# waczjoan/gaussian-mesh-splatting

Measured on AMD Instinct MI355X. Metric: train iters/s (fwd+bwd raster) @800×800, 300k Gaussians; HBM GB/s vs roofline, higher is better.
Workload: dtype f32

## Files before the change

gaussian-mesh-splatting_amd/csrc/blend_micro.hip:

```cpp
#include <stdlib.h>

#include "gms_common.h"
#include "gms_blend.h"
#include "gms_segments.h"

namespace gms {

struct MPix {
    int xi, yi, tid, b; bool inside; float xf, yf;
    static __device__ __forceinline__ MPix of_tile(const BlendGrid &g, int tile);
};

__device__ __forceinline__ MPix micro_pixel(const BlendGrid &g, int tx, int ty, int b, int li)
{
    MPix p;
    p.b = b;
    p.xi = tx * TILE + (b & 3) * 4 + (li & 3);
    p.yi = ty * TILE + (b >> 2) * 4 + (li >> 2);
    p.inside = p.xi < g.W && p.yi < g.H;
    p.xf = (float)p.xi; p.yf = (float)p.yi;
    p.tid = b * 16 + li;
    return p;
}

__device__ __forceinline__ uint32_t max4rows(uint32_t v)
{
    const uint32_t a = (uint32_t)__builtin_amdgcn_readlane((int)v, 0), b = (uint32_t)__builtin_amdgcn_readlane((int)v, 16);
    const uint32_t c = (uint32_t)__builtin_amdgcn_readlane((int)v, 32), d = (uint32_t)__builtin_amdgcn_readlane((int)v, 48);
    return max(max(a, b), max(c, d));
}

constexpr int LMAX = 256;

__device__ __forceinline__ MPix MPix::of_tile(const BlendGrid &g, int tile)
{
    return micro_pixel(g, tile % g.gx, tile / g.gx, (int)(threadIdx.x >> 4), (int)(threadIdx.x & 15));
}

__global__ void __launch_bounds__(BLOCK) micro_tloc_check_kernel(BlendGrid g)
{
    tile_dead_check<MPix>(g);
}

__global__ void __launch_bounds__(BLOCK) micro_finalize_kernel(BlendGrid g, BlendFwdOut o)
{
    const uint32_t order_blocks = g.bwd_order ? UNIT_ORDER_CLASSES : 0u;
    if (blockIdx.x < order_blocks) {
        __shared__ UnitOrderLds S;
        const uint32_t n = min(g.unit_first[g.T], g.max_units);
        unit_order_partition(blockIdx.x, n, blend_grid_units(g.max_units), g.order_on ? UNIT_ORDER_CLASSES : 0u,
                             [&](uint32_t i) { return (uint32_t)g.unit_cost[i]; },
                             [&](uint32_t i) { const uint2 r = reinterpret_cast<const uint2 *>(g.unit_tile)[4 * (size_t)i + 2]; return r.x != r.y; },
                             g.bwd_order, S);
        return;
    }
    finalize_tile<8, MPix>(g, o, (int)(blockIdx.x - order_blocks));
}

struct Phases {
    unsigned long long *buf; bool on;
    __device__ __forceinline__ Phases(const BlendGrid &g, uint32_t bit = 1024u) : buf(nullptr), on(false)
    {
        if (dbg_on(g, bit) && g.dbg_buf) {
            buf = g.dbg_buf + 8ull * 65536ull * (threadIdx.x >> 6) + 8ull * (blockIdx.x & 65535u);
            on = (threadIdx.x & 63) == 0;
        }
    }
    __device__ __forceinline__ void mark(int k) { if (on) buf[k] = wall_clock64(); }
    __device__ __forceinline__ void value(int k, unsigned long long v) { if (on) buf[k] = v; }
};

template <int CTRL>
__device__ __forceinline__ float dpp_mov(float v)
{
    return __builtin_bit_cast(float, __builtin_amdgcn_update_dpp(0, __builtin_bit_cast(int, v), CTRL, 0xf, 0xf, false));
}

#define GMS_BANK_PAIR(D, A, B, CTRL, LO, HI)                                                                                          \
    "v_add_f32_dpp " D ", " A ", " A " " CTRL " row_mask:0xf bank_mask:" LO "\n\tv_add_f32_dpp " D ", " B ", " B " " CTRL " row_mask:0xf bank_mask:" HI "\n\t"
template <bool NINE>
__device__ __forceinline__ void bank_stage_ror8(const float *v, float (&u)[5])
{
    if (NINE)
        asm volatile("s_nop 1\n\t"
                     GMS_BANK_PAIR("%0", "%5", "%10", "row_ror:8", "0x3", "0xc") GMS_BANK_PAIR("%1", "%6", "%11", "row_ror:8", "0x3", "0xc")
                     GMS_BANK_PAIR("%2", "%7", "%12", "row_ror:8", "0x3", "0xc") GMS_BANK_PAIR("%3", "%8", "%13", "row_ror:8", "0x3", "0xc")
                     "v_add_f32_dpp %4, %9, %9 row_ror:8 row_mask:0xf bank_mask:0x3\n\t"
                     : "=&v"(u[0]), "=&v"(u[1]), "=&v"(u[2]), "=&v"(u[3]), "=&v"(u[4])
                     : "v"(v[0]), "v"(v[1]), "v"(v[2]), "v"(v[3]), "v"(v[4]), "v"(v[5]), "v"(v[6]), "v"(v[7]), "v"(v[8]));
    else
        asm volatile("s_nop 1\n\t"
                     GMS_BANK_PAIR("%0", "%5", "%10", "row_ror:8", "0x3", "0xc") GMS_BANK_PAIR("%1", "%6", "%11", "row_ror:8", "0x3", "0xc")
                     GMS_BANK_PAIR("%2", "%7", "%12", "row_ror:8", "0x3", "0xc") GMS_BANK_PAIR("%3", "%8", "%13", "row_ror:8", "0x3", "0xc")
                     GMS_BANK_PAIR("%4", "%9", "%14", "row_ror:8", "0x3", "0xc")
                     : "=&v"(u[0]), "=&v"(u[1]), "=&v"(u[2]), "=&v"(u[3]), "=&v"(u[4])
                     : "v"(v[0]), "v"(v[1]), "v"(v[2]), "v"(v[3]), "v"(v[4]), "v"(v[5]), "v"(v[6]), "v"(v[7]), "v"(v[8]), "v"(v[9]));
}
__device__ __forceinline__ void bank_stage_half_mirror(float a0, float b0, float a1, float b1, float &w0, float &w1)
{
    asm volatile("s_nop 1\n\t"
                 GMS_BANK_PAIR("%0", "%2", "%3", "row_half_mirror", "0x5", "0xa") GMS_BANK_PAIR("%1", "%4", "%5", "row_half_mirror", "0x5", "0xa")
                 : "=&v"(w0), "=&v"(w1) : "v"(a0), "v"(b0), "v"(a1), "v"(b1));
}

template <bool NINE = false>
__device__ __forceinline__ float row_reduce10(const float *v, bool b1, bool b0)
{
    float u[5];
    bank_stage_ror8<NINE>(v, u);
    float w0, w1;
    bank_stage_half_mirror(u[0], u[3], u[1], u[4], w0, w1);
    const float w2 = u[2] + dpp_mov<0x141>(u[2]);
    const float x0 = (b1 ? w1 : w0) + dpp_mov<0x4E>(b1 ? w0 : w1);
    const float x1 = w2 + dpp_mov<0x4E>(w2);
    return (b0 ? x1 : x0) + dpp_mov<0xB1>(b0 ? x0 : x1);
}

template <int CTRL, int ROW_MASK = 0xf>
__device__ __forceinline__ float dpp_max(float v)
{
    return fmaxf(v, __builtin_bit_cast(float, __builtin_amdgcn_update_dpp(0, __builtin_bit_cast(int, v), CTRL, ROW_MASK, 0xf, false)));
}
__device__ __forceinline__ float wave_max_to_lane63(float v)
{
    v = dpp_max<0xB1>(v); v = dpp_max<0x4E>(v); v = dpp_max<0x141>(v); v = dpp_max<0x140>(v);
    v = dpp_max<0x142, 0xa>(v); v = dpp_max<0x143, 0xc>(v);
    return v;
}

template <bool WITHD> struct RecTail { using type = float2; };
template <> struct RecTail<false> { using type = float; };
__device__ __forceinline__ void set_tail(float2 &d, float b, float invd) { d = make_float2(b, invd); }
__device__ __forceinline__ void set_tail(float &d, float b, float) { d = b; }
__device__ __forceinline__ float2 get_tail(const float2 &d) { return d; }
__device__ __forceinline__ float2 get_tail(const float &d) { return make_float2(d, 0.f); }
struct __attribute__((aligned(16))) WideTail { float2 v; float2 unused; };
__device__ __forceinline__ void set_tail(WideTail &d, float b, float invd) { d.v = make_float2(b, invd); }
__device__ __forceinline__ float2 get_tail(const WideTail &d) { return d.v; }
template <bool WITHD, bool WIDE> struct RecTailSel { using type = typename RecTail<WITHD>::type; };
template <> struct RecTailSel<true, true> { using type = WideTail; };
template <bool WITHD, bool WIDE = false>
struct UnitRecsT {
    float4 ra[LMAX];
    float4 rb[LMAX];
    typename RecTailSel<WITHD, WIDE>::type rc[LMAX];
    uint8_t list[16][LMAX];
    uint16_t ocnt[16];
    uint8_t order[16];
    uint8_t wcnt4[16][4];
};
using UnitRecs = UnitRecsT<true, true>;

template <int NE> __device__ __forceinline__ uint32_t list_load(const uint8_t *lst, uint32_t pos);
template <> __device__ __forceinline__ uint32_t list_load<2>(const uint8_t *lst, uint32_t pos) { return *reinterpret_cast<const uint16_t *>(lst + pos); }
template <> __device__ __forceinline__ uint32_t list_load<4>(const uint8_t *lst, uint32_t pos) { return *reinterpret_cast<const uint32_t *>(lst + pos); }

template <bool FILTER, bool WITHD, bool WIDE>
__device__ __forceinline__ uint32_t unit_stage(const BlendGrid &g, const Unit &u, UnitRecsT<WITHD, WIDE> &S, const SplatRec *rec, uint32_t *cmax_out,
                                               Phases *ph = nullptr)
{
    const int tid = threadIdx.x, lane = tid & 63, wave = tid >> 6;
    const uint32_t cn = u.end - u.beg;
    uint16_t *mm = g.mmask;
    uint32_t mask = 0, id = 0;
    float cm = 0.f;
    if ((uint32_t)tid < cn) {
        id = reinterpret_cast<const uint32_t *>(g.keys)[2 * (size_t)(u.beg + tid)];
        if (!FILTER) mask = mm[u.beg + tid];
        const SplatRec r = rec[id];
        if (FILTER) { mask = block_mask(r, (float)(u.tx * TILE), (float)(u.ty * TILE)); mm[u.beg + tid] = (uint16_t)mask; }
        S.ra[tid] = r.q0; S.rb[tid] = r.q1; set_tail(S.rc[tid], r.q2.x, r.q2.y);
        cm = fmaxf(fmaxf(fabsf(r.q1.z), fabsf(r.q1.w)), fabsf(r.q2.x));
    } else if (tid < LMAX) {
        S.ra[tid] = make_float4(0.f, 0.f, 0.f, 0.f); S.rb[tid] = make_float4(0.f, 0.f, 0.f, 0.f); set_tail(S.rc[tid], 0.f, 0.f);
    }
    if (cmax_out) {
        cm = wave_max_to_lane63(cm);
        if (lane == 63 && cm > 0.f) atomicMax(cmax_out, __float_as_uint(cm));
    }
    if (GMS_EXPERIMENTS && ph) { __builtin_amdgcn_s_waitcnt(0); ph->mark(3); }
    uint64_t bal[16];
    uint32_t mycnt = 0;
#pragma unroll
    for (int b = 0; b < 16; b++) {
        bal[b] = __ballot((mask >> b) & 1u);
        const uint32_t n = (uint32_t)__builtin_popcountll(bal[b]);
        asm("v_writelane_b32 %0, %1, %2" : "+v"(mycnt) : "s"(n), "n"(b));
    }
    if (lane < 16) S.wcnt4[lane][wave] = (uint8_t)mycnt;
    __syncthreads();
    if (GMS_EXPERIMENTS && ph) ph->mark(4);
    const uint32_t w4 = *reinterpret_cast<const uint32_t *>(&S.wcnt4[lane & 15][0]);
    const uint32_t basev = __builtin_amdgcn_sad_u8(w4 & ((1u << (8 * wave)) - 1u), 0u, 0u);
#pragma unroll
    for (int b = 0; b < 16; b++) {
        const uint32_t base = (uint32_t)__builtin_amdgcn_readlane((int)basev, b);
        const uint32_t pos = __builtin_amdgcn_mbcnt_hi((uint32_t)(bal[b] >> 32), __builtin_amdgcn_mbcnt_lo((uint32_t)bal[b], base));
        if ((mask >> b) & 1u) S.list[b][pos] = (uint8_t)tid;
    }
    if (tid < 16) {
        const uint32_t c = __builtin_amdgcn_sad_u8(w4, 0u, 0u);
        uint32_t rank = 0;
#pragma unroll
        for (int s0 = 0; s0 < 16; s0++) {
            const uint32_t cs = (uint32_t)__builtin_amdgcn_readlane((int)c, s0);
            rank += (cs > c || (cs == c && s0 < tid)) ? 1u : 0u;
        }
        S.order[rank] = (uint8_t)tid; S.ocnt[rank] = (uint16_t)c;
        if (FILTER && rank == 0) g.unit_cost[u.idx] = (uint16_t)c;
    }
    __syncthreads();
    return id;
}

constexpr uint32_t LAST_NONE = 0x7fffffffu;
constexpr int REM_STOPPED = -0x40000000;
template <int E>
__device__ __forceinline__ void fwd_step_exec(float pw, float al, float cr, float cg, float cb, float cd, float &T, float &C0, float &C1, float &C2,
                                              float &Dp, int &rem, uint32_t &last)
{
    uint64_t sv; float tmp, w;
    asm volatile("s_mov_b64 %[sv], exec\n\t"
                 "v_cmpx_lt_i32_e32 vcc, %[e], %[rem]\n\t"
                 "v_cmpx_ge_f32_e32 vcc, 0, %[pw]\n\t"
                 "v_cmpx_le_f32_e32 vcc, %[amin], %[al]\n\t"
                 "v_sub_f32_e32 %[tmp], 1.0, %[al]\n\t"
                 "v_mul_f32_e32 %[tmp], %[T], %[tmp]\n\t"
                 "v_cmp_ngt_f32_e32 vcc, %[tmin], %[tmp]\n\t"
                 "v_cndmask_b32_e32 %[rem], %[stopped], %[rem], vcc\n\t"
                 "s_and_b64 exec, exec, vcc\n\t"
                 "v_mul_f32_e32 %[w], %[al], %[T]\n\t"
                 "v_fmac_f32_e32 %[C0], %[cr], %[w]\n\t"
                 "v_fmac_f32_e32 %[C1], %[cg], %[w]\n\t"
                 "v_fmac_f32_e32 %[C2], %[cb], %[w]\n\t"
                 "v_fmac_f32_e32 %[Dp], %[cd], %[w]\n\t"
                 "v_mov_b32_e32 %[T], %[tmp]\n\t"
                 "v_sub_u32_e32 %[last], %[e], %[rem]\n\t"
                 "s_mov_b64 exec, %[sv]"
                 : [sv] "=&s"(sv), [tmp] "=&v"(tmp), [w] "=&v"(w), [T] "+v"(T), [C0] "+v"(C0), [C1] "+v"(C1), [C2] "+v"(C2), [Dp] "+v"(Dp),
                   [rem] "+v"(rem), [last] "+v"(last)
                 : [e] "n"(E), [pw] "v"(pw), [al] "v"(al), [amin] "s"(ALPHA_MIN), [tmin] "s"(T_MIN), [stopped] "v"(REM_STOPPED), [cr] "v"(cr), [cg] "v"(cg), [cb] "v"(cb), [cd] "v"(cd)
                 : "vcc");
}
template <int E>
__device__ __forceinline__ void tloc_step_exec(float pw, float al, float &Tl, int rem)
{
    uint64_t sv; float tmp;
    asm volatile("s_mov_b64 %[sv], exec\n\t"
                 "v_cmpx_lt_i32_e32 vcc, %[e], %[rem]\n\t"
                 "v_cmpx_ge_f32_e32 vcc, 0, %[pw]\n\t"
                 "v_cmpx_le_f32_e32 vcc, %[amin], %[al]\n\t"
                 "v_sub_f32_e32 %[tmp], 1.0, %[al]\n\t"
                 "v_mul_f32_e32 %[Tl], %[Tl], %[tmp]\n\t"
                 "s_mov_b64 exec, %[sv]"
                 : [sv] "=&s"(sv), [tmp] "=&v"(tmp), [Tl] "+v"(Tl)
                 : [e] "n"(E), [pw] "v"(pw), [al] "v"(al), [amin] "s"(ALPHA_MIN), [rem] "v"(rem)
                 : "vcc");
}
template <int NE, int E = 0> struct StepUnroll {
    template <class F> static __device__ __forceinline__ void run(F &&f) { f(std::integral_constant<int, E>{}); StepUnroll<NE, E + 1>::run(f); }
};
template <int NE> struct StepUnroll<NE, NE> { template <class F> static __device__ __forceinline__ void run(F &&) {} };

template <int NE>
__device__ __forceinline__ void micro_tloc_unit(const BlendGrid &g, const Unit &u, const UnitRecs &S, int phase, int q)
{
    const int lane = threadIdx.x & 63, row = lane >> 4, li = lane & 15;
    const MPix p = micro_pixel(g, u.tx, u.ty, (int)S.order[4 * q + row], li);
    float *dst = g.seg_state + (size_t)(u.slot0 + u.seg) * SEG_FLOATS + SEG_TLOC * TILE_PIX + p.tid;
    const uint32_t cnt = S.ocnt[4 * q + row];
    const uint8_t *lst = S.list[p.b];
    float Tl = 1.f;
    (void)phase;
    int rem = p.inside ? (int)cnt : 0;
    static_assert(LMAX % NE == 0, "a trip reads NE list bytes at a multiple of NE below the row's count");
    if (__builtin_amdgcn_ballot_w64(rem > 0) != 0ull) do {
        const uint32_t ep = list_load<NE>(lst, 0);
        float al[NE], pw[NE];
#pragma unroll
        for (int e = 0; e < NE; e++) {
            const uint32_t ent = (ep >> (8 * e)) & 0xffu;
            const float4 r0 = S.ra[ent];
            const float2 r1 = *reinterpret_cast<const float2 *>(&S.rb[ent]);
            const float dx = r0.x - p.xf, dy = r0.y - p.yf;
            pw[e] = pair_power(r0.z, r0.w, r1.x, dx, dy);
            al[e] = fminf(ALPHA_MAX, r1.y * __expf(pw[e]));
        }
        StepUnroll<NE>::run([&](auto e) { tloc_step_exec<decltype(e)::value>(pw[decltype(e)::value], al[decltype(e)::value], Tl, rem); });
        rem -= NE; lst += NE;
    } while (__builtin_amdgcn_ballot_w64(rem > 0 && !(Tl < T_MIN)) != 0ull);
    *dst = Tl;
}

template <int NE>
__device__ __forceinline__ void micro_fwd_unit(const BlendGrid &g, const BlendFwdOut &o, const Unit &u, const UnitRecs &S, int q)
{
    const int lane = threadIdx.x & 63, row = lane >> 4, li = lane & 15;
    const MPix p = micro_pixel(g, u.tx, u.ty, (int)S.order[4 * q + row], li);
    const uint32_t cnt = S.ocnt[4 * q + row];
    const uint8_t *lst = S.list[p.b];
    const uint32_t posbase = (uint32_t)u.seg * u.L;

    float T = prefix_transmittance<8>(g, u, p.tid);
    const bool dead_on_entry = T < T_MIN;
    float C0 = 0.f, C1 = 0.f, C2 = 0.f, Dp = 0.f;
    uint32_t last_rel = LAST_NONE;
    int rem = (!p.inside || dead_on_entry) ? 0 : (int)cnt;

    static_assert(LMAX % NE == 0, "a trip reads NE list bytes at a multiple of NE below the row's count");
    if (__builtin_amdgcn_ballot_w64(rem > 0) != 0ull) do {
        const uint32_t ep = list_load<NE>(lst, 0);
        float al[NE], pw[NE]; float2 cg[NE], cb[NE];
#pragma unroll
        for (int e = 0; e < NE; e++) {
            const uint32_t ent = (ep >> (8 * e)) & 0xffu;
            const float4 r0 = S.ra[ent], r1 = S.rb[ent];
            cb[e] = get_tail(S.rc[ent]);
            cg[e] = make_float2(r1.z, r1.w);
            const float dx = r0.x - p.xf, dy = r0.y - p.yf;
            pw[e] = pair_power(r0.z, r0.w, r1.x, dx, dy);
            al[e] = fminf(ALPHA_MAX, r1.y * __expf(pw[e]));
        }
        StepUnroll<NE>::run([&](auto e) {
            constexpr int E = decltype(e)::value;
            fwd_step_exec<E>(pw[E], al[E], cg[E].x, cg[E].y, cb[E].x, cb[E].y, T, C0, C1, C2, Dp, rem, last_rel);
        });
        rem -= NE; lst += NE;
    } while (__builtin_amdgcn_ballot_w64(rem > 0) != 0ull);
    const bool done = !p.inside || dead_on_entry || rem < REM_STOPPED / 2;
    const uint32_t last = last_rel == LAST_NONE ? 0u : posbase + cnt + 1u + last_rel;
    if (u.nseg == 1) write_pixel(g, o, p, T, last, C0, C1, C2, Dp);
    else store_partials(g, u, p.tid, T, last, C0, C1, C2, Dp, dead_on_entry, done);
}

template <int NE>
__global__ void __launch_bounds__(BLOCK) micro_head_kernel(BlendGrid g, BlendFwdOut o, int phase)
{
    __shared__ UnitRecs S;
    Phases ph(g, 2048u);
    ph.mark(0);
    Unit u;
    if (!load_unit_at(g, u, blockIdx.x >> 3, blockIdx.x & 7u)) return;
    const bool walk = u.seg == 0 ? phase <= 0
                                 : (u.nseg > 1 && u.seg != u.nseg - 1 && (phase < 0 || (u.seg < tloc_head(u.L)) == (phase == 0)));
    if (!walk) return;
    if (u.end == u.beg) {
        write_pixel(g, o, micro_pixel(g, u.tx, u.ty, (int)(threadIdx.x >> 4), (int)(threadIdx.x & 15)), 1.f, 0u, 0.f, 0.f, 0.f, 0.f);
        return;
    }
    if (u.seg > 0 && phase == 1 && g.tile_dead[u.tile]) {
        if (threadIdx.x < u.end - u.beg) g.mmask[u.beg + threadIdx.x] = 0;
        if (threadIdx.x == 0) g.unit_cost[u.idx] = 0;
        g.seg_state[(size_t)(u.slot0 + u.seg) * SEG_FLOATS + SEG_TLOC * TILE_PIX + threadIdx.x] = 0.f;
        return;
    }
    unit_stage<true>(g, u, S, o.rec, g.tile_cmax + u.tile, &ph);
    ph.mark(1);
    const int q = (int)(((threadIdx.x >> 6) + (blockIdx.x >> 3)) & 3u);
    if (u.seg == 0) micro_fwd_unit<NE>(g, o, u, S, q);
    else micro_tloc_unit<NE>(g, u, S, phase, q);
    ph.value(6, u.seg == 0 ? 1ull : 2ull);
    ph.value(7, ((unsigned long long)u.idx << 40) | ((unsigned long long)(u.end - u.beg) << 28) | ((unsigned long long)u.nseg << 14) | (unsigned long long)u.seg);
    ph.value(2, (unsigned long long)(g.tile_offset[u.tile + 1] - g.tile_offset[u.tile]));
    ph.mark(5);
}

template <int NE>
__global__ void __launch_bounds__(BLOCK) micro_fwd_kernel(BlendGrid g, BlendFwdOut o)
{
    __shared__ UnitRecs S;
    Phases ph(g, 4096u);
    ph.mark(0);
    Unit u;
    if (!load_unit_at(g, u, blockIdx.x >> 3, blockIdx.x & 7u)) return;
    if (u.seg == 0) return;
    if (u.seg == u.nseg - 1) unit_stage<true>(g, u, S, o.rec, g.tile_cmax + u.tile, &ph);
    else unit_stage<false>(g, u, S, o.rec, g.tile_cmax + u.tile, &ph);
    ph.mark(1);
    const int q = (int)(((threadIdx.x >> 6) + (blockIdx.x >> 3)) & 3u);
    micro_fwd_unit<NE>(g, o, u, S, q);
    ph.value(6, u.seg == u.nseg - 1 ? 3ull : 4ull);
    ph.value(7, ((unsigned long long)u.idx << 40) | ((unsigned long long)(u.end - u.beg) << 28) | ((unsigned long long)u.nseg << 14) | (unsigned long long)u.seg);
    ph.value(2, (unsigned long long)(g.tile_offset[u.tile + 1] - g.tile_offset[u.tile]));
    ph.mark(5);
}


template <bool INVD, int NE, int FAULT, bool DET = false>
__global__ void __launch_bounds__(BLOCK) micro_bwd_kernel(BlendGrid g, BlendBwdArgs a)
{
    constexpr int NF = INVD ? 10 : 9;
    __shared__ UnitRecsT<INVD> S;
    __shared__ __attribute__((aligned(8))) unsigned char table_mem[LMAX * NF * 8];
    __shared__ uint32_t tile_max[5];
    long long *const fxt = reinterpret_cast<long long *>(table_mem);
    uint32_t *const uid = reinterpret_cast<uint32_t *>(S.rc);
    Phases ph(g);
    ph.mark(0);
    Unit u;
    if (!load_unit_at(g, u, blockIdx.x >> 3, blockIdx.x & 7u, g.bwd_order)) return;
    if (u.end <= u.beg) return;
    if (u.end - u.beg > (uint32_t)LMAX) return;
    for (int k = threadIdx.x; k < LMAX * NF; k += BLOCK) fxt[k] = 0ll;
    if (threadIdx.x < 5) tile_max[threadIdx.x] = 0u;
    const uint32_t my_id = unit_stage<false, INVD>(g, u, S, a.rec, nullptr);
    ph.mark(1);
    const int q = (int)(((threadIdx.x >> 6) + (blockIdx.x >> 3)) & 3u);
    const int lane = threadIdx.x & 63, row = lane >> 4, li = lane & 15;
    const MPix p = micro_pixel(g, u.tx, u.ty, (int)S.order[4 * q + row], li);
    const BwdPixel bp = bwd_pixel<INVD>(g, a, p);
    const uint32_t last = bp.last;
    const float dp0 = bp.dp0, dp1 = bp.dp1, dp2 = bp.dp2, dinvd = bp.dinvd, Tfinal_bgdot = bp.Tfinal_bgdot;
    FxTile fx = {0, 0, 0, 0, 0};
    const float tx0 = (float)(u.tx * TILE), ty0 = (float)(u.ty * TILE);
    const float4 mine = S.ra[threadIdx.x & 0xffu];
    const bool real = (uint32_t)threadIdx.x < u.end - u.beg;
    const float m_d1 = wave_max_to_lane63((fabsf(dp0) + fabsf(dp1)) + fabsf(dp2));
    const float m_x = wave_max_to_lane63(real ? fmaxf(fabsf(mine.x - tx0), fabsf(mine.x - tx0 - 15.f)) + 1.f : 1.f);
    const float m_y = wave_max_to_lane63(real ? fmaxf(fabsf(mine.y - ty0), fabsf(mine.y - ty0 - 15.f)) + 1.f : 1.f);
    const float m_dd = INVD ? wave_max_to_lane63(fabsf(dinvd)) : 0.f;
    const float m_op = wave_max_to_lane63(real ? fabsf(S.rb[threadIdx.x & 0xffu].y) : 0.f);
    if (lane == 63) {
        atomicMax(&tile_max[0], __float_as_uint(m_d1)); if (INVD) atomicMax(&tile_max[1], __float_as_uint(m_dd));
        atomicMax(&tile_max[2], __float_as_uint(m_x)); atomicMax(&tile_max[3], __float_as_uint(m_y));
        atomicMax(&tile_max[4], __float_as_uint(m_op));
    }
    __syncthreads();
    const float D1 = __uint_as_float(tile_max[0]), Dd = INVD ? __uint_as_float(tile_max[1]) : 0.f;
    const float cmax = __uint_as_float(g.tile_cmax[u.tile]);
    const float bgm = fmaxf(fmaxf(fabsf(a.bg[0]), fabsf(a.bg[1])), fabsf(a.bg[2]));
    fx.eK = fx_exp(32.f * ((cmax + bgm) * D1 + 5.f * Dd)) + fx_exp(__uint_as_float(tile_max[4]));
    fx.eX = fx_exp(__uint_as_float(tile_max[2]));
    fx.eY = fx_exp(__uint_as_float(tile_max[3]));
    fx.eCol = fx_exp(32.f * D1);
    fx.eId = fx_exp(32.f * Dd);
    const uint32_t posbase = (uint32_t)u.seg * u.L;
    const uint32_t cn = u.end - u.beg;
    const uint32_t cnt = S.ocnt[4 * q + row];
    const uint8_t *lst = S.list[p.b];
    const uint32_t lrel = last > posbase ? min(last - posbase, cnt) : 0u;
    uint32_t top = lrel;
    top = max(top, (uint32_t)__shfl_xor((int)top, 8)); top = max(top, (uint32_t)__shfl_xor((int)top, 4));
    top = max(top, (uint32_t)__shfl_xor((int)top, 2)); top = max(top, (uint32_t)__shfl_xor((int)top, 1));
    const uint32_t maxtop = max4rows(top);
    ph.value(6, maxtop);

    if (maxtop > 0) {
    BwdState st8 = {bp.Tfinal, 0.f, 0.f, 0.f, 0.f};
    bwd_restart<INVD, FAULT, 8>(g, u, p.tid, st8);
    ph.mark(2);

    const bool b1 = (li & 2) != 0, b0 = (li & 1) != 0;
    int afield;
    switch (li) {
    case 0: afield = GRAD_MX; break;
    case 8: afield = GRAD_OP; break;
    case 4: afield = GRAD_CB; break;
    case 12: afield = GRAD_B; break;
    case 2: afield = GRAD_MY; break;
    case 10: afield = GRAD_R; break;
    case 6: afield = GRAD_CC; break;
    case 14: afield = GRAD_ID; break;
    case 1: afield = GRAD_CA; break;
    default: afield = GRAD_G; break;
    }
    const bool alane = (li & 1) == 0 ? (li != 14 || INVD) : (li == 1 || li == 9);
    int fcx, fcy, fkind;
    fx_field_kind(afield, fcx, fcy, fkind);
    const int fxbase = fx_field_base(fx, fcx, fcy, fkind);
    const FxScale fxs = fx_prepare(fx_scale_exp(fxbase, 126u));

    for (int g0 = (int)(((maxtop + NE - 1u) / NE) * NE) - NE; g0 >= 0; g0 -= NE) {
        const uint32_t ep = list_load<NE>(lst, (uint32_t)g0);
        bool act[NE]; float dx[NE], dy[NE], G[NE], al[NE]; float4 r1[NE]; float2 r2[NE]; uint32_t se[NE];
        bool anyact = false;
#pragma unroll
        for (int e = 0; e < NE; e++) {
            const uint32_t pos = (uint32_t)g0 + (uint32_t)(NE - 1 - e);
            se[e] = (ep >> (8 * (NE - 1 - e))) & 0xffu;
            const float4 r0 = S.ra[se[e]];
            r1[e] = S.rb[se[e]]; r2[e] = get_tail(S.rc[se[e]]);
            dx[e] = r0.x - p.xf; dy[e] = r0.y - p.yf;
            const float pw = pair_power(r0.z, r0.w, r1[e].x, dx[e], dy[e]);
            G[e] = __expf(pw);
            al[e] = fminf(ALPHA_MAX, r1[e].y * G[e]);
            act[e] = pos < lrel && pw <= 0.f && al[e] >= ALPHA_MIN;
            anyact = anyact || act[e];
        }
        if (!__any(anyact)) continue;
        float y[NE];
        {
            float v[NE][10];
#pragma unroll
            for (int e = 0; e < NE; e++) {
                const float4 q2 = make_float4(r2[e].x, r2[e].y, 0.f, 0.f);
                bwd_step<INVD>(st8, act[e], r1[e], q2, dx[e], dy[e], G[e], al[e], dp0, dp1, dp2, dinvd, Tfinal_bgdot, v[e]);
            }
#pragma unroll
            for (int e = 0; e < NE; e++) y[e] = row_reduce10<!INVD>(v[e], b1, b0);
        }
        long long val[NE];
#pragma unroll
        for (int e = 0; e < NE; e++) val[e] = fx_from_float(y[e], fxs);
#pragma unroll
        for (int e = 0; e < NE; e++)
            if (alane && y[e] != 0.f)
                atomicAdd(reinterpret_cast<unsigned long long *>(fxt) + se[e] * (uint32_t)NF + (uint32_t)afield, (unsigned long long)val[e]);
    }
    }
    ph.mark(3);
    __syncthreads();
    ph.mark(4);
    if ((uint32_t)threadIdx.x < cn) uid[threadIdx.x] = my_id;
    __syncthreads();
    if (!DET) {
        constexpr int EPS = BLOCK / NF;
        const int f = (int)threadIdx.x % NF;
        int cx, cy, kind;
        fx_field_kind(f, cx, cy, kind);
        const int kexp = fx_scale_exp(fx_field_base(fx, cx, cy, kind), 126u);
        if ((int)threadIdx.x < EPS * NF) {
            for (uint32_t e = threadIdx.x / NF; e < cn; e += EPS) {
                const long long sv = fxt[e * (uint32_t)NF + (uint32_t)f];
                if (sv != 0ll)
                    unsafeAtomicAdd(a.accum + (size_t)uid[e] * GRAD_STRIDE + f, fx_to_float(sv, kexp));
            }
        }
    } else {
        const int f = threadIdx.x & 15;
        int cx, cy, kind;
        fx_field_kind(f, cx, cy, kind);
        for (uint32_t e = threadIdx.x >> 4; e < cn; e += BLOCK / 16) {
            const long long sv = f < NF ? fxt[e * (uint32_t)NF + (uint32_t)f] : 0ll;
            a.part[(size_t)(u.beg + e) * GRAD_STRIDE + f] = sv != 0ll ? fx_to_float(sv, fx_scale_exp(fx_field_base(fx, cx, cy, kind), 126u)) : 0.f;
        }
    }
    ph.value(7, ((unsigned long long)u.idx << 40) | ((unsigned long long)(u.end - u.beg) << 28) | ((unsigned long long)u.nseg << 14) | (unsigned long long)u.seg);
    ph.mark(5);
}

const BlendFamily &micro_family()
{
    static const BlendFamily f = {
        micro_head_kernel<4>, micro_tloc_check_kernel, micro_fwd_kernel<4>, micro_finalize_kernel,
        {{micro_bwd_kernel<false, 2, 0>, micro_bwd_kernel<false, 2, 0, true>, micro_bwd_kernel<false, 2, 2>},
         {micro_bwd_kernel<true, 2, 0>, micro_bwd_kernel<true, 2, 0, true>, micro_bwd_kernel<true, 2, 0>}},
        1u, BLOCK, 2048u | 4096u, 1024u, 1u, "micro_head", "micro_fwd", "micro_finalize", "micro_bwd"};
    return f;
}

}
```

Before: 3140.

## Trim unit staging and backward prologue reductions with DPP and per-wave maxima

Several micro-optimizations land together. Wave max now uses unsigned-integer DPP on clamped floats. The ballot and list-scatter loops are skipped for waves with no mask hits, and the 16-way rank uses DPP rotates on a packed key instead of readlane. Shared-memory atomicMax tile maxima are replaced by per-wave slots that are reduced after the barrier. The fx table zeroing covers only the live records, the row max uses DPP instead of shuffles, and the afield switch becomes a packed constant lookup. Each piece targets prologue overhead in the backward blend kernel, and the changes add some risk around clamping negative values and tie ordering in the rank.

```diff
diff --git a/gaussian-mesh-splatting_amd/csrc/blend_micro.hip b/gaussian-mesh-splatting_amd/csrc/blend_micro.hip
--- a/gaussian-mesh-splatting_amd/csrc/blend_micro.hip
+++ b/gaussian-mesh-splatting_amd/csrc/blend_micro.hip
@@ -117,15 +117,20 @@
 }
 
 template <int CTRL, int ROW_MASK = 0xf>
-__device__ __forceinline__ float dpp_max(float v)
-{
-    return fmaxf(v, __builtin_bit_cast(float, __builtin_amdgcn_update_dpp(0, __builtin_bit_cast(int, v), CTRL, ROW_MASK, 0xf, false)));
+__device__ __forceinline__ uint32_t dpp_umax(uint32_t v)
+{
+    return max(v, (uint32_t)__builtin_amdgcn_update_dpp(0, (int)v, CTRL, ROW_MASK, 0xf, false));
+}
+__device__ __forceinline__ uint32_t row_umax(uint32_t v)
+{
+    v = dpp_umax<0xB1>(v); v = dpp_umax<0x4E>(v); v = dpp_umax<0x141>(v); v = dpp_umax<0x140>(v);
+    return v;
 }
 __device__ __forceinline__ float wave_max_to_lane63(float v)
 {
-    v = dpp_max<0xB1>(v); v = dpp_max<0x4E>(v); v = dpp_max<0x141>(v); v = dpp_max<0x140>(v);
-    v = dpp_max<0x142, 0xa>(v); v = dpp_max<0x143, 0xc>(v);
-    return v;
+    uint32_t b = row_umax(__float_as_uint(fmaxf(v, 0.f)));
+    b = dpp_umax<0x142, 0xa>(b); b = dpp_umax<0x143, 0xc>(b);
+    return __uint_as_float(b);
 }
 
 template <bool WITHD> struct RecTail { using type = float2; };
@@ -151,6 +156,11 @@
 };
 using UnitRecs = UnitRecsT<true, true>;
 
+template <int NE, int E = 0> struct StepUnroll {
+    template <class F> static __device__ __forceinline__ void run(F &&f) { f(std::integral_constant<int, E>{}); StepUnroll<NE, E + 1>::run(f); }
+};
+template <int NE> struct StepUnroll<NE, NE> { template <class F> static __device__ __forceinline__ void run(F &&) {} };
+
 template <int NE> __device__ __forceinline__ uint32_t list_load(const uint8_t *lst, uint32_t pos);
 template <> __device__ __forceinline__ uint32_t list_load<2>(const uint8_t *lst, uint32_t pos) { return *reinterpret_cast<const uint16_t *>(lst + pos); }
 template <> __device__ __forceinline__ uint32_t list_load<4>(const uint8_t *lst, uint32_t pos) { return *reinterpret_cast<const uint32_t *>(lst + pos); }
@@ -181,31 +191,39 @@
     if (GMS_EXPERIMENTS && ph) { __builtin_amdgcn_s_waitcnt(0); ph->mark(3); }
     uint64_t bal[16];
     uint32_t mycnt = 0;
-#pragma unroll
-    for (int b = 0; b < 16; b++) {
-        bal[b] = __ballot((mask >> b) & 1u);
-        const uint32_t n = (uint32_t)__builtin_popcountll(bal[b]);
-        asm("v_writelane_b32 %0, %1, %2" : "+v"(mycnt) : "s"(n), "n"(b));
+    const bool wave_hits = __ballot(mask != 0u) != 0ull;
+#pragma unroll
+    for (int b = 0; b < 16; b++) bal[b] = 0ull;
+    if (wave_hits) {
+#pragma unroll
+        for (int b = 0; b < 16; b++) {
+            bal[b] = __ballot((mask >> b) & 1u);
+            const uint32_t n = (uint32_t)__builtin_popcountll(bal[b]);
+            asm("v_writelane_b32 %0, %1, %2" : "+v"(mycnt) : "s"(n), "n"(b));
+        }
     }
     if (lane < 16) S.wcnt4[lane][wave] = (uint8_t)mycnt;
     __syncthreads();
     if (GMS_EXPERIMENTS && ph) ph->mark(4);
     const uint32_t w4 = *reinterpret_cast<const uint32_t *>(&S.wcnt4[lane & 15][0]);
     const uint32_t basev = __builtin_amdgcn_sad_u8(w4 & ((1u << (8 * wave)) - 1u), 0u, 0u);
-#pragma unroll
-    for (int b = 0; b < 16; b++) {
-        const uint32_t base = (uint32_t)__builtin_amdgcn_readlane((int)basev, b);
-        const uint32_t pos = __builtin_amdgcn_mbcnt_hi((uint32_t)(bal[b] >> 32), __builtin_amdgcn_mbcnt_lo((uint32_t)bal[b], base));
-        if ((mask >> b) & 1u) S.list[b][pos] = (uint8_t)tid;
+    if (wave_hits) {
+#pragma unroll
+        for (int b = 0; b < 16; b++) {
+            if (bal[b] == 0ull) continue;
+            const uint32_t base = (uint32_t)__builtin_amdgcn_readlane((int)basev, b);
+            const uint32_t pos = __builtin_amdgcn_mbcnt_hi((uint32_t)(bal[b] >> 32), __builtin_amdgcn_mbcnt_lo((uint32_t)bal[b], base));
+            if ((mask >> b) & 1u) S.list[b][pos] = (uint8_t)tid;
+        }
     }
     if (tid < 16) {
         const uint32_t c = __builtin_amdgcn_sad_u8(w4, 0u, 0u);
+        const uint32_t key = (c << 4) | (15u - (uint32_t)tid);
         uint32_t rank = 0;
-#pragma unroll
-        for (int s0 = 0; s0 < 16; s0++) {
-            const uint32_t cs = (uint32_t)__builtin_amdgcn_readlane((int)c, s0);
-            rank += (cs > c || (cs == c && s0 < tid)) ? 1u : 0u;
-        }
+        StepUnroll<16, 1>::run([&](auto k) {
+            constexpr int ROR = 0x120 + decltype(k)::value;
+            rank += (uint32_t)__builtin_amdgcn_mov_dpp((int)key, ROR, 0xf, 0xf, false) > key ? 1u : 0u;
+        });
         S.order[rank] = (uint8_t)tid; S.ocnt[rank] = (uint16_t)c;
         if (FILTER && rank == 0) g.unit_cost[u.idx] = (uint16_t)c;
     }
@@ -257,11 +275,6 @@
                  : [e] "n"(E), [pw] "v"(pw), [al] "v"(al), [amin] "s"(ALPHA_MIN), [rem] "v"(rem)
                  : "vcc");
 }
-template <int NE, int E = 0> struct StepUnroll {
-    template <class F> static __device__ __forceinline__ void run(F &&f) { f(std::integral_constant<int, E>{}); StepUnroll<NE, E + 1>::run(f); }
-};
-template <int NE> struct StepUnroll<NE, NE> { template <class F> static __device__ __forceinline__ void run(F &&) {} };
-
 template <int NE>
 __device__ __forceinline__ void micro_tloc_unit(const BlendGrid &g, const Unit &u, const UnitRecs &S, int phase, int q)
 {
@@ -392,7 +405,8 @@
     constexpr int NF = INVD ? 10 : 9;
     __shared__ UnitRecsT<INVD> S;
     __shared__ __attribute__((aligned(8))) unsigned char table_mem[LMAX * NF * 8];
-    __shared__ uint32_t tile_max[5];
+    __shared__ uint4 wave_max[BLOCK / WAVE];
+    __shared__ uint32_t wave_max_dd[BLOCK / WAVE];
     long long *const fxt = reinterpret_cast<long long *>(table_mem);
     uint32_t *const uid = reinterpret_cast<uint32_t *>(S.rc);
     Phases ph(g);
@@ -401,8 +415,7 @@
     if (!load_unit_at(g, u, blockIdx.x >> 3, blockIdx.x & 7u, g.bwd_order)) return;
     if (u.end <= u.beg) return;
     if (u.end - u.beg > (uint32_t)LMAX) return;
-    for (int k = threadIdx.x; k < LMAX * NF; k += BLOCK) fxt[k] = 0ll;
-    if (threadIdx.x < 5) tile_max[threadIdx.x] = 0u;
+    for (uint32_t k = threadIdx.x; k < (u.end - u.beg) * (uint32_t)NF; k += BLOCK) fxt[k] = 0ll;
     const uint32_t my_id = unit_stage<false, INVD>(g, u, S, a.rec, nullptr);
     ph.mark(1);
     const int q = (int)(((threadIdx.x >> 6) + (blockIdx.x >> 3)) & 3u);
@@ -416,22 +429,26 @@
     const float4 mine = S.ra[threadIdx.x & 0xffu];
     const bool real = (uint32_t)threadIdx.x < u.end - u.beg;
     const float m_d1 = wave_max_to_lane63((fabsf(dp0) + fabsf(dp1)) + fabsf(dp2));
-    const float m_x = wave_max_to_lane63(real ? fmaxf(fabsf(mine.x - tx0), fabsf(mine.x - tx0 - 15.f)) + 1.f : 1.f);
-    const float m_y = wave_max_to_lane63(real ? fmaxf(fabsf(mine.y - ty0), fabsf(mine.y - ty0 - 15.f)) + 1.f : 1.f);
     const float m_dd = INVD ? wave_max_to_lane63(fabsf(dinvd)) : 0.f;
-    const float m_op = wave_max_to_lane63(real ? fabsf(S.rb[threadIdx.x & 0xffu].y) : 0.f);
+    float m_x = 0.f, m_y = 0.f, m_op = 0.f;
+    if (__ballot(real) != 0ull) {
+        m_x = wave_max_to_lane63(real ? fmaxf(fabsf(mine.x - tx0), fabsf(mine.x - tx0 - 15.f)) + 1.f : 1.f);
+        m_y = wave_max_to_lane63(real ? fmaxf(fabsf(mine.y - ty0), fabsf(mine.y - ty0 - 15.f)) + 1.f : 1.f);
+        m_op = wave_max_to_lane63(real ? fabsf(S.rb[threadIdx.x & 0xffu].y) : 0.f);
+    }
     if (lane == 63) {
-        atomicMax(&tile_max[0], __float_as_uint(m_d1)); if (INVD) atomicMax(&tile_max[1], __float_as_uint(m_dd));
-        atomicMax(&tile_max[2], __float_as_uint(m_x)); atomicMax(&tile_max[3], __float_as_uint(m_y));
-        atomicMax(&tile_max[4], __float_as_uint(m_op));
+        wave_max[threadIdx.x >> 6] = make_uint4(__float_as_uint(m_d1), __float_as_uint(m_x), __float_as_uint(m_y), __float_as_uint(m_op));
+        if (INVD) wave_max_dd[threadIdx.x >> 6] = __float_as_uint(m_dd);
     }
     __syncthreads();
-    const float D1 = __uint_as_float(tile_max[0]), Dd = INVD ? __uint_as_float(tile_max[1]) : 0.f;
+    const uint4 wm0 = wave_max[0], wm1 = wave_max[1], wm2 = wave_max[2], wm3 = wave_max[3];
+    const float D1 = __uint_as_float(max(max(wm0.x, wm1.x), max(wm2.x, wm3.x)));
+    const float Dd = INVD ? __uint_as_float(max(max(wave_max_dd[0], wave_max_dd[1]), max(wave_max_dd[2], wave_max_dd[3]))) : 0.f;
     const float cmax = __uint_as_float(g.tile_cmax[u.tile]);
     const float bgm = fmaxf(fmaxf(fabsf(a.bg[0]), fabsf(a.bg[1])), fabsf(a.bg[2]));
-    fx.eK = fx_exp(32.f * ((cmax + bgm) * D1 + 5.f * Dd)) + fx_exp(__uint_as_float(tile_max[4]));
-    fx.eX = fx_exp(__uint_as_float(tile_max[2]));
-    fx.eY = fx_exp(__uint_as_float(tile_max[3]));
+    fx.eK = fx_exp(32.f * ((cmax + bgm) * D1 + 5.f * Dd)) + fx_exp(__uint_as_float(max(max(wm0.w, wm1.w), max(wm2.w, wm3.w))));
+    fx.eX = fx_exp(__uint_as_float(max(max(wm0.y, wm1.y), max(wm2.y, wm3.y))));
+    fx.eY = fx_exp(__uint_as_float(max(max(wm0.z, wm1.z), max(wm2.z, wm3.z))));
     fx.eCol = fx_exp(32.f * D1);
     fx.eId = fx_exp(32.f * Dd);
     const uint32_t posbase = (uint32_t)u.seg * u.L;
@@ -439,10 +456,7 @@
     const uint32_t cnt = S.ocnt[4 * q + row];
     const uint8_t *lst = S.list[p.b];
     const uint32_t lrel = last > posbase ? min(last - posbase, cnt) : 0u;
-    uint32_t top = lrel;
-    top = max(top, (uint32_t)__shfl_xor((int)top, 8)); top = max(top, (uint32_t)__shfl_xor((int)top, 4));
-    top = max(top, (uint32_t)__shfl_xor((int)top, 2)); top = max(top, (uint32_t)__shfl_xor((int)top, 1));
-    const uint32_t maxtop = max4rows(top);
+    const uint32_t maxtop = max4rows(row_umax(lrel));
     ph.value(6, maxtop);
 
     if (maxtop > 0) {
@@ -451,19 +465,11 @@
     ph.mark(2);
 
     const bool b1 = (li & 2) != 0, b0 = (li & 1) != 0;
-    int afield;
-    switch (li) {
-    case 0: afield = GRAD_MX; break;
-    case 8: afield = GRAD_OP; break;
-    case 4: afield = GRAD_CB; break;
-    case 12: afield = GRAD_B; break;
-    case 2: afield = GRAD_MY; break;
-    case 10: afield = GRAD_R; break;
-    case 6: afield = GRAD_CC; break;
-    case 14: afield = GRAD_ID; break;
-    case 1: afield = GRAD_CA; break;
-    default: afield = GRAD_G; break;
-    }
+    constexpr uint64_t AFIELD = (uint64_t)GRAD_MX << 0 | (uint64_t)GRAD_CA << 4 | (uint64_t)GRAD_MY << 8 | (uint64_t)GRAD_G << 12 |
+                                (uint64_t)GRAD_CB << 16 | (uint64_t)GRAD_G << 20 | (uint64_t)GRAD_CC << 24 | (uint64_t)GRAD_G << 28 |
+                                (uint64_t)GRAD_OP << 32 | (uint64_t)GRAD_G << 36 | (uint64_t)GRAD_R << 40 | (uint64_t)GRAD_G << 44 |
+                                (uint64_t)GRAD_B << 48 | (uint64_t)GRAD_G << 52 | (uint64_t)GRAD_ID << 56 | (uint64_t)GRAD_G << 60;
+    const int afield = (int)(((li < 8 ? (uint32_t)AFIELD : (uint32_t)(AFIELD >> 32)) >> (4 * (li & 7))) & 15u);
     const bool alane = (li & 1) == 0 ? (li != 14 || INVD) : (li == 1 || li == 9);
     int fcx, fcy, fkind;
     fx_field_kind(afield, fcx, fcy, fkind);
```

Measured after the change: 3223 (median of 6 runs). +2.6%, better.
